# stdstu12/YUME

Hardware: AMD Instinct MI355X
Metric: denoise-steps/sec (Yume-5B 720P, 33-frame latent) (higher is better)
Workload: dtype bf16; 1 GPU; Yume-5B-720P random-init, 33-frame 704x1280 clip (latent 48x13x44x80, FramePack lfz=8, L=9460), ODE Euler steps of a 50-step shift-7 schedule, no CFG, one chain per GPU; num_layers=30, parallelism=dp1 (independent chains, replicated weights)

## Files before the change

### include/yume_hip.h

```cpp
#ifndef YUME_HIP_H
#define YUME_HIP_H

#include <stdint.h>

#ifdef __cplusplus
extern "C" {
#endif

#define YUME_OK 0
#define YUME_EINVAL (-1)
#define YUME_ELAUNCH (-2)
#define YUME_EUNSUP (-3)

const char* yume_last_error(void);
#define YUME_ABI_VERSION 9
int yume_abi_version(void);
const char* yume_target_arch(void);

int64_t yume_counter_workspace_bytes(void);
int yume_counter_workspace_init(void* ptr, int64_t bytes, void* stream);

int yume_calibrate_mfma(int64_t iters, int64_t workgroups, void* ticks, void* sink, void* stream);

int yume_adaln_modulate(const float* x, int64_t ldx, int64_t T, int64_t C, float eps,
// ... 13 lines not shown
};
int yume_gemm_bf16(const void* A, int64_t lda, const void* W, int64_t ldw, const float* bias,
                   int64_t M, int64_t N, int64_t K, int epi,
                   void* out, int64_t ldo,
                   const float* gate, int64_t gate_stride, const int32_t* row_idx,
                   void* outT, int64_t ldt, int64_t n_split,
                   int variant, void* stream);

int64_t yume_gemm_workspace_bytes(void);
int yume_gemm_bf16_ws(const void* A, int64_t lda, const void* W, int64_t ldw, const float* bias,
                      int64_t M, int64_t N, int64_t K, int epi,
                      void* out, int64_t ldo,
                      const float* gate, int64_t gate_stride, const int32_t* row_idx,
                      void* outT, int64_t ldt, int64_t n_split,
                      int variant, void* workspace, int64_t workspace_bytes, void* stream);

int yume_quant_rows_e4m3(const void* x, int64_t ldx, int64_t R, int64_t K, void* q, int64_t ldq, float* scale, void* stream);
int yume_gemm_f8(const void* Aq, int64_t lda, const float* sa, const void* Wq, int64_t ldw, const float* sw,
                 const float* bias, int64_t M, int64_t N, int64_t K, int epi, void* out, int64_t ldo,
                 const float* gate, int64_t gate_stride, const int32_t* row_idx, void* stream);
int yume_gemm_f8_splitt(const void* Aq, int64_t lda, const float* sa, const void* Wq, int64_t ldw, const float* sw,
                        const float* bias, int64_t M, int64_t N, int64_t K,
                        void* out, int64_t ldo, void* outT, int64_t ldt, int64_t n_split, void* stream);

int yume_adaln_modulate_e4m3(const float* x, int64_t ldx, int64_t T, int64_t C, float eps, const float* mul,
                             const float* add, int64_t tab_stride, const int32_t* row_idx, int add_one,
                             void* q, int64_t ldq, float* scale, void* stream);
int yume_gemm_f8_mxout(const void* Aq, int64_t lda, const float* sa, const void* Wq, int64_t ldw, const float* sw,
                       const float* bias, int64_t M, int64_t N, int64_t K, int epi, void* out, int64_t ldo,
                       void* eo, int64_t ldeo, void* stream);
int yume_gemm_f8_mx(const void* Aq, int64_t lda, const void* ea, int64_t ldea, const void* Wq, int64_t ldw, const float* sw,
                    const float* bias, int64_t M, int64_t N, int64_t K, int epi, void* out, int64_t ldo,
                    const float* gate, int64_t gate_stride, const int32_t* row_idx, void* stream);

int yume_rmsnorm_rope(void* buf, int64_t ld, int64_t T, int64_t C, int nparts,
                      const float* w, float eps, const float* rope, int64_t D, void* stream);
int yume_rmsnorm_rows_periodic(void* buf, int64_t ld, int64_t T, int64_t C, const float* w, int64_t wperiod, float eps,
                               void* stream);

#define YUME_ATTN_Q_PRESCALED 0x100
#define YUME_ATTN_KV_PADDED 0x200
int yume_attn_fwd(const void* Q, int64_t ldq, const void* K, int64_t ldk, const void* Vt, int64_t ldvt,
                  void* O, int64_t ldo, int64_t Lq, int64_t Lk, int64_t H, float scale,
                  int accumulate, int variant, void* stream);
int64_t yume_attn_workspace_bytes(int64_t Lq, int64_t Lk, int64_t H);
int yume_attn_fwd_ws(const void* Q, int64_t ldq, const void* K, int64_t ldk, const void* Vt, int64_t ldvt,
                     void* O, int64_t ldo, int64_t Lq, int64_t Lk, int64_t H, float scale,
                     int accumulate, int variant, void* workspace, int64_t workspace_bytes, void* stream);
int yume_attn_fwd_kw(const void* Q, int64_t ldq, const void* K, int64_t ldk, const void* Vt, int64_t ldvt,
                     void* O, int64_t ldo, int64_t Lq, int64_t Lk, int64_t H, float scale,
                     int accumulate, int variant, void* workspace, int64_t workspace_bytes, float last_key_weight, void* stream);
int yume_attn_fwd_seg(const void* Q, int64_t ldq, const void* const* K, int64_t ldk, const void* const* Vt, int64_t ldvt,
                      void* O, int64_t ldo, int64_t nseg, int64_t Lq_seg, int64_t seg_pitch, const int64_t* Lk, int64_t H,
                      float scale, int accumulate, int variant, const float* last_key_weight, void* stream);
int64_t yume_attn_batch_workspace_bytes(int64_t nseg, int64_t Lq_seg, int64_t Lk_seg, int64_t H);
int yume_attn_fwd_batch(const void* Q, int64_t ldq, const void* K, int64_t ldk, const void* Vt, int64_t ldvt,
                        void* O, int64_t ldo, int64_t nseg, int64_t Lq_seg, int64_t q_pitch,
                        int64_t Lk_seg, int64_t k_pitch, int64_t H, float scale, int accumulate, int variant,
                        void* workspace, int64_t workspace_bytes, void* stream);

int yume_linear_smallm_f32(const float* in, int64_t R, int64_t K, const void* W, int w_bf16,
                           const float* bias, int64_t N, int in_act, int out_act,
                           const float* add_table, float* out, void* stream);

int yume_sinusoidal_embed(const double* t, const int32_t* t_index, int64_t R, int64_t dim,
                          float* out, void* stream);
// ... 59 lines not shown
```

### yume_amd/_lib.py

```python
import ctypes
import os
from ctypes import c_void_p, c_int, c_int64, c_float, c_char_p

_HERE = os.path.dirname(os.path.abspath(__file__))
LIB_PATH = os.environ.get("YUME_HIP_LIB") or os.path.join(_HERE, "lib", "libyume_hip.so")

_P, _I, _L, _F = c_void_p, c_int, c_int64, c_float

SIGNATURES = {
    "yume_last_error": [],
    "yume_abi_version": [],
    "yume_target_arch": [],
    "yume_counter_workspace_bytes": [],
    "yume_counter_workspace_init": [_P, _L, _P],
    "yume_calibrate_mfma": [_L, _L, _P, _P, _P],
    "yume_adaln_modulate": [_P, _L, _L, _L, _F, _P, _P, _L, _P, _I, _P, _L, _I, _P],
    "yume_adaln_modulate_e4m3": [_P, _L, _L, _L, _F, _P, _P, _L, _P, _I, _P, _L, _P, _P],
    "yume_gemm_bf16": [_P, _L, _P, _L, _P, _L, _L, _L, _I, _P, _L, _P, _L, _P, _P, _L, _L, _I, _P],
    "yume_gemm_workspace_bytes": [],
    "yume_gemm_bf16_ws": [_P, _L, _P, _L, _P, _L, _L, _L, _I, _P, _L, _P, _L, _P, _P, _L, _L, _I, _P, _L, _P],
    "yume_quant_rows_e4m3": [_P, _L, _L, _L, _P, _L, _P, _P],
    "yume_gemm_f8": [_P, _L, _P, _P, _L, _P, _P, _L, _L, _L, _I, _P, _L, _P, _L, _P, _P],
    "yume_gemm_f8_splitt": [_P, _L, _P, _P, _L, _P, _P, _L, _L, _L, _P, _L, _P, _L, _L, _P],
    "yume_gemm_f8_mxout": [_P, _L, _P, _P, _L, _P, _P, _L, _L, _L, _I, _P, _L, _P, _L, _P],
    "yume_gemm_f8_mx": [_P, _L, _P, _L, _P, _L, _P, _P, _L, _L, _L, _I, _P, _L, _P, _L, _P, _P],
    "yume_rmsnorm_f32": [_P, _L, _L, _L, _F, _P, _P, _L, _P],
    "yume_gemm_bf16_batched": [_P, _L, _L, _P, _L, _L, _L, _L, _L, _I, _P, _L, _L, _L, _I, _P],
    "yume_gemm_splitk_workspace_bytes": [_L, _L, _I],
    "yume_gemm_bf16_splitk": [_P, _L, _P, _L, _P, _L, _L, _L, _I, _P, _L, _I, _P, _P],
    "yume_softmax_bias_rows": [_P, _L, _L, _L, _L, _P, _L, _P, _L, _L, _P],
    "yume_rmsnorm_rows_periodic": [_P, _L, _L, _L, _P, _L, _F, _P],
    "yume_rmsnorm_rope": [_P, _L, _L, _L, _I, _P, _F, _P, _L, _P],
    "yume_attn_fwd": [_P, _L, _P, _L, _P, _L, _P, _L, _L, _L, _L, _F, _I, _I, _P],
    "yume_attn_workspace_bytes": [_L, _L, _L],
    "yume_attn_fwd_ws": [_P, _L, _P, _L, _P, _L, _P, _L, _L, _L, _L, _F, _I, _I, _P, _L, _P],
    "yume_attn_fwd_kw": [_P, _L, _P, _L, _P, _L, _P, _L, _L, _L, _L, _F, _I, _I, _P, _L, _F, _P],
    "yume_attn_fwd_seg": [_P, _L, _P, _L, _P, _L, _P, _L, _L, _L, _L, _P, _L, _F, _I, _I, _P, _P],
    "yume_attn_batch_workspace_bytes": [_L, _L, _L, _L],
    "yume_attn_fwd_batch": [_P, _L, _P, _L, _P, _L, _P, _L, _L, _L, _L, _L, _L, _L, _F, _I, _I, _P, _L, _P],
    "yume_linear_smallm_f32": [_P, _L, _L, _P, _I, _P, _L, _I, _I, _P, _P, _P],
    "yume_sinusoidal_embed": [_P, _P, _L, _L, _P, _P],
    "yume_modulation_table": [_P, _P, _L, _L, _L, _P, _P],
    "yume_patch_gather": [_P, _I, _L, _L, _L, _L, _L, _L, _L, _L, _P, _L, _P],
    "yume_unpatchify": [_P, _L, _L, _L, _L, _L, _L, _L, _P, _P],
    "yume_cast_bf16": [_P, _L, _L, _L, _L, _P, _L, _P],
    "yume_transpose_bf16": [_P, _I, _L, _L, _L, _P, _L, _P],
    "yume_conv3d_cl": [_P, _P, _L, _L, _L, _L, _L, _P, _L, _P, _L, _I, _I, _I, _I, _I, _I, _I, _I, _I, _I, _L, _L, _L, _I, _P, _L,
                       _P, _L, _P, _P],
    "yume_vae_rmsnorm_silu": [_P, _L, _L, _L, _P, _P, _I, _P, _L, _P],
    "yume_vae_dupup_add": [_P, _L, _L, _L, _L, _L, _P, _L, _L, _L, _I, _I, _I, _P],
    "yume_vae_avgdown_add": [_P, _L, _L, _L, _L, _L, _P, _L, _L, _I, _I, _P],
    "yume_softmax_rows": [_P, _L, _L, _L, _F, _P, _L, _P],
    "yume_vae_pack_input": [_P, _I, _L, _L, _L, _L, _I, _P, _P, _P, _L, _P],
    "yume_frames_u8": [_P, _L, _L, _L, _L, _P, _P],
    "yume_frames_u8_trunc": [_P, _L, _L, _L, _L, _P, _P],
    "yume_vae_unpack_output": [_P, _L, _L, _L, _L, _L, _I, _P, _P, _F, _F, _P, _P],
}
_RES = {"yume_last_error": c_char_p, "yume_target_arch": c_char_p, "yume_gemm_splitk_workspace_bytes": c_int64, "yume_attn_workspace_bytes": c_int64,
# ... 35 lines not shown
```

### yume_amd/csrc/gemm_f8.hip

```cpp
#include "gemm_f8.hpp"

using namespace gemm_core;

namespace {
bool f8_log() {
    static const bool on = [] { const char* v = getenv("YUME_GEMM_LOG"); return v && atoi(v) != 0; }();
    return on;
}
}

extern "C" int yume_gemm_f8(const void* Aq, int64_t lda, const float* sa, const void* Wq, int64_t ldw, const float* sw, const float* bias,
                            int64_t M, int64_t N, int64_t K, int epi, void* out, int64_t ldo, const float* gate, int64_t gate_stride,
                            const int32_t* row_idx, void* stream) {
    if (epi != YUME_EPI_BF16 && epi != YUME_EPI_BF16_GELU && epi != YUME_EPI_F32 && epi != YUME_EPI_RESID) {
        yume_set_error("gemm_f8: epilogue %d is not implemented (BF16, GELU, F32, RESID are)", epi);
        return YUME_EUNSUP;
    }
    YUME_REQUIRE(Aq && Wq && sa && sw && out, "gemm_f8: NULL pointer");
    YUME_REQUIRE(M > 0 && N > 0 && K > 0, "gemm_f8: empty problem M=%lld N=%lld K=%lld", (long long)M, (long long)N, (long long)K);
    YUME_REQUIRE(M < (1ll << 31) && N < (1ll << 31) && K < (1ll << 31), "gemm_f8: dimension too large");
    YUME_REQUIRE((K % gemm_f8::F8_BK) == 0, "gemm_f8: K=%lld must be a multiple of %d", (long long)K, gemm_f8::F8_BK);
    YUME_REQUIRE((N % 4) == 0, "gemm_f8: N=%lld must be a multiple of 4", (long long)N);
    YUME_REQUIRE((lda % 16) == 0 && (ldw % 16) == 0 && lda >= K && ldw >= K, "gemm_f8: lda/ldw must be multiples of 16 (16-byte rows) and >= K");
    YUME_REQUIRE((ldo % 4) == 0 && ldo >= N, "gemm_f8: ldo must be a multiple of 4 and >= N");
    YUME_REQUIRE(((uintptr_t)Aq % 16) == 0 && ((uintptr_t)Wq % 16) == 0 && ((uintptr_t)out % 16) == 0 && ((uintptr_t)sw % 16) == 0 &&
                 ((uintptr_t)sa % 4) == 0 && (bias == nullptr || ((uintptr_t)bias % 16) == 0),
                 "gemm_f8: Aq, Wq, out, sw and bias must be 16-byte aligned");
    if (epi == YUME_EPI_RESID)
        YUME_REQUIRE(gate == nullptr || ((gate_stride % 4) == 0 && ((uintptr_t)gate % 16) == 0), "gemm_f8: gate must be 16-byte aligned, gate_stride a multiple of 4");
    Problem p = {};
    p.M = (int)M; p.N = (int)N; p.K = (int)K;
    gemm_f8::F8Args f = {};
    f.A = (const unsigned char*)Aq; f.lda = lda; f.sa = sa;
    f.W = (const unsigned char*)Wq; f.ldw = ldw; f.sw = sw;
    Epilogue e = {};
    e.bias = bias;
    e.out = out; e.ldo = ldo;
    e.gate = gate; e.gate_stride = gate_stride; e.row_idx = row_idx;
    if (f8_log())
        fprintf(stderr, "[gemm_f8] f8 M=%lld N=%lld K=%lld epi=%d lda=%lld ldw=%lld ldo=%lld\n", (long long)M, (long long)N, (long long)K, epi,
                (long long)lda, (long long)ldw, (long long)ldo);
    return gemm_f8::launch_f8(epi, p, f, e, (hipStream_t)stream);
}

extern "C" int yume_gemm_f8_splitt(const void* Aq, int64_t lda, const float* sa, const void* Wq, int64_t ldw, const float* sw, const float* bias,
                                   int64_t M, int64_t N, int64_t K, void* out, int64_t ldo, void* outT, int64_t ldt, int64_t n_split,
                                   void* stream) {
    YUME_REQUIRE(Aq && Wq && sa && sw, "gemm_f8_splitt: NULL pointer");
    YUME_REQUIRE(M > 0 && N > 0 && K > 0, "gemm_f8_splitt: empty problem M=%lld N=%lld K=%lld", (long long)M, (long long)N, (long long)K);
    YUME_REQUIRE(M < (1ll << 31) && N < (1ll << 31) && K < (1ll << 31), "gemm_f8_splitt: dimension too large");
    YUME_REQUIRE((K % gemm_f8::F8_BK) == 0, "gemm_f8_splitt: K=%lld must be a multiple of %d", (long long)K, gemm_f8::F8_BK);
    YUME_REQUIRE((N % 4) == 0, "gemm_f8_splitt: N=%lld must be a multiple of 4", (long long)N);
    YUME_REQUIRE((lda % 16) == 0 && (ldw % 16) == 0 && lda >= K && ldw >= K, "gemm_f8_splitt: lda/ldw must be multiples of 16 (16-byte rows) and >= K");
    YUME_REQUIRE(n_split >= 0 && n_split <= N && (n_split % 256) == 0, "gemm_f8_splitt: n_split=%lld must be a multiple of 256 in [0, N=%lld]",
                 (long long)n_split, (long long)N);
    YUME_REQUIRE(n_split == 0 || out != nullptr, "gemm_f8_splitt: NULL out with n_split > 0");
    YUME_REQUIRE(n_split == 0 || ((ldo % 4) == 0 && ldo >= n_split), "gemm_f8_splitt: ldo=%lld must be a multiple of 4 and >= n_split", (long long)ldo);
    YUME_REQUIRE(n_split == N || outT != nullptr, "gemm_f8_splitt: NULL outT with n_split < N");
    YUME_REQUIRE(n_split == N || ((ldt % 8) == 0 && ldt >= M), "gemm_f8_splitt: ldt=%lld must be a multiple of 8 and >= M", (long long)ldt);
    YUME_REQUIRE(((uintptr_t)Aq % 16) == 0 && ((uintptr_t)Wq % 16) == 0 && ((uintptr_t)out % 16) == 0 && ((uintptr_t)outT % 16) == 0 &&
                 ((uintptr_t)sw % 16) == 0 && ((uintptr_t)sa % 4) == 0 && (bias == nullptr || ((uintptr_t)bias % 16) == 0),
                 "gemm_f8_splitt: Aq, Wq, out, outT, sw and bias must be 16-byte aligned");
    Problem p = {};
    p.M = (int)M; p.N = (int)N; p.K = (int)K;
    gemm_f8::F8Args f = {};
    f.A = (const unsigned char*)Aq; f.lda = lda; f.sa = sa;
    f.W = (const unsigned char*)Wq; f.ldw = ldw; f.sw = sw;
    Epilogue e = {};
    e.bias = bias;
    e.out = out; e.ldo = ldo;
    e.outT = (unsigned short*)outT; e.ldt = ldt; e.n_split = (int)n_split;
    if (f8_log())
        fprintf(stderr, "[gemm_f8] f8 M=%lld N=%lld K=%lld epi=%d lda=%lld ldw=%lld ldo=%lld ldt=%lld n_split=%lld\n", (long long)M, (long long)N,
                (long long)K, (int)YUME_EPI_BF16_SPLITT, (long long)lda, (long long)ldw, (long long)ldo, (long long)ldt, (long long)n_split);
    return gemm_f8::launch_f8(YUME_EPI_BF16_SPLITT, p, f, e, (hipStream_t)stream);
}

extern "C" int yume_gemm_f8_mxout(const void* Aq, int64_t lda, const float* sa, const void* Wq, int64_t ldw, const float* sw, const float* bias,
                                  int64_t M, int64_t N, int64_t K, int epi, void* out, int64_t ldo, void* eo, int64_t ldeo, void* stream) {
    if (epi != YUME_EPI_MX_GELU) {
        yume_set_error("gemm_f8_mxout: epilogue %d is not implemented (MX_GELU is)", epi);
        return YUME_EUNSUP;
    }
    YUME_REQUIRE(Aq && Wq && sa && sw && out && eo, "gemm_f8_mxout: NULL pointer");
    YUME_REQUIRE(M > 0 && N > 0 && K > 0, "gemm_f8_mxout: empty problem M=%lld N=%lld K=%lld", (long long)M, (long long)N, (long long)K);
    YUME_REQUIRE(M < (1ll << 31) && N < (1ll << 31) && K < (1ll << 31), "gemm_f8_mxout: dimension too large");
    YUME_REQUIRE((K % gemm_f8::F8_BK) == 0, "gemm_f8_mxout: K=%lld must be a multiple of %d", (long long)K, gemm_f8::F8_BK);
    YUME_REQUIRE((N % 32) == 0, "gemm_f8_mxout: N=%lld must be a multiple of 32 (one scale byte per 32 columns)", (long long)N);
    YUME_REQUIRE((lda % 16) == 0 && (ldw % 16) == 0 && lda >= K && ldw >= K, "gemm_f8_mxout: lda/ldw must be multiples of 16 (16-byte rows) and >= K");
    YUME_REQUIRE((ldo % 4) == 0 && ldo >= N, "gemm_f8_mxout: ldo must be a multiple of 4 and >= N");
    YUME_REQUIRE(ldeo >= N / 32, "gemm_f8_mxout: ldeo=%lld must be >= N / 32", (long long)ldeo);
    YUME_REQUIRE(((uintptr_t)Aq % 16) == 0 && ((uintptr_t)Wq % 16) == 0 && ((uintptr_t)out % 16) == 0 && ((uintptr_t)sw % 16) == 0 &&
                 ((uintptr_t)sa % 4) == 0 && (bias == nullptr || ((uintptr_t)bias % 16) == 0),
                 "gemm_f8_mxout: Aq, Wq, out, sw and bias must be 16-byte aligned");
    Problem p = {};
    p.M = (int)M; p.N = (int)N; p.K = (int)K;
    gemm_f8::F8Args f = {};
    f.A = (const unsigned char*)Aq; f.lda = lda; f.sa = sa;
    f.W = (const unsigned char*)Wq; f.ldw = ldw; f.sw = sw;
    f.eo = (unsigned char*)eo; f.ldeo = ldeo;
    Epilogue e = {};
    e.bias = bias;
    e.out = out; e.ldo = ldo;
    if (f8_log())
        fprintf(stderr, "[gemm_f8] f8 M=%lld N=%lld K=%lld epi=%d lda=%lld ldw=%lld ldo=%lld ldeo=%lld\n", (long long)M, (long long)N, (long long)K, epi,
                (long long)lda, (long long)ldw, (long long)ldo, (long long)ldeo);
    return gemm_f8::launch_f8(epi, p, f, e, (hipStream_t)stream);
}

extern "C" int yume_gemm_f8_mx(const void* Aq, int64_t lda, const void* ea, int64_t ldea, const void* Wq, int64_t ldw, const float* sw,
                               const float* bias, int64_t M, int64_t N, int64_t K, int epi, void* out, int64_t ldo, const float* gate,
                               int64_t gate_stride, const int32_t* row_idx, void* stream) {
    if (epi != YUME_EPI_F32 && epi != YUME_EPI_RESID) {
        yume_set_error("gemm_f8_mx: epilogue %d is not implemented (F32, RESID are)", epi);
        return YUME_EUNSUP;
    }
    YUME_REQUIRE(Aq && Wq && ea && sw && out, "gemm_f8_mx: NULL pointer");
    YUME_REQUIRE(M > 0 && N > 0 && K > 0, "gemm_f8_mx: empty problem M=%lld N=%lld K=%lld", (long long)M, (long long)N, (long long)K);
    YUME_REQUIRE(M < (1ll << 31) && N < (1ll << 31) && K < (1ll << 31), "gemm_f8_mx: dimension too large");
    YUME_REQUIRE((K % gemm_f8::F8_BK) == 0, "gemm_f8_mx: K=%lld must be a multiple of %d", (long long)K, gemm_f8::F8_BK);
    YUME_REQUIRE((N % 4) == 0, "gemm_f8_mx: N=%lld must be a multiple of 4", (long long)N);
    YUME_REQUIRE((lda % 16) == 0 && (ldw % 16) == 0 && lda >= K && ldw >= K, "gemm_f8_mx: lda/ldw must be multiples of 16 (16-byte rows) and >= K");
    YUME_REQUIRE((ldea % 16) == 0 && ldea >= K / 32, "gemm_f8_mx: ldea=%lld must be a multiple of 16 and >= K / 32", (long long)ldea);
    YUME_REQUIRE((ldo % 4) == 0 && ldo >= N, "gemm_f8_mx: ldo must be a multiple of 4 and >= N");
    YUME_REQUIRE(((uintptr_t)Aq % 16) == 0 && ((uintptr_t)Wq % 16) == 0 && ((uintptr_t)out % 16) == 0 && ((uintptr_t)sw % 16) == 0 &&
                 ((uintptr_t)ea % 16) == 0 && (bias == nullptr || ((uintptr_t)bias % 16) == 0),
                 "gemm_f8_mx: Aq, ea, Wq, out, sw and bias must be 16-byte aligned");
    if (epi == YUME_EPI_RESID)
        YUME_REQUIRE(gate == nullptr || ((gate_stride % 4) == 0 && ((uintptr_t)gate % 16) == 0), "gemm_f8_mx: gate must be 16-byte aligned, gate_stride a multiple of 4");
    Problem p = {};
    p.M = (int)M; p.N = (int)N; p.K = (int)K;
    gemm_f8::F8Args f = {};
    f.A = (const unsigned char*)Aq; f.lda = lda;
    f.W = (const unsigned char*)Wq; f.ldw = ldw; f.sw = sw;
    f.ea = (const unsigned char*)ea; f.ldea = ldea;
    Epilogue e = {};
    e.bias = bias;
    e.out = out; e.ldo = ldo;
    e.gate = gate; e.gate_stride = gate_stride; e.row_idx = row_idx;
    if (f8_log())
        fprintf(stderr, "[gemm_f8] mx M=%lld N=%lld K=%lld epi=%d lda=%lld ldea=%lld ldw=%lld ldo=%lld\n", (long long)M, (long long)N, (long long)K, epi,
                (long long)lda, (long long)ldea, (long long)ldw, (long long)ldo);
    return gemm_f8::launch_f8_mx(epi, p, f, e, (hipStream_t)stream);
}
```

### yume_amd/csrc/gemm_f8.hpp

```cpp
#pragma once
#include "gemm_w4.hpp"

namespace gemm_f8 {
using namespace gemm_core;

typedef __attribute__((ext_vector_type(8))) int i32x8;

constexpr int F8_BK = 128;
constexpr int F8_NTHR = 256;
constexpr int F8_OPER = 256 * F8_BK;
constexpr int F8_BUF = 2 * F8_OPER;
constexpr int F8_LDS = 2 * F8_BUF;

struct F8Args {
    const unsigned char* A; int64_t lda; const float* sa;
    const unsigned char* W; int64_t ldw; const float* sw;
    const unsigned char* ea; int64_t ldea;
    unsigned char* eo; int64_t ldeo;
};

constexpr int EPI_MX_GELU = YUME_EPI_MX_GELU;

__device__ __forceinline__ void f8_stage(const unsigned char* const (&ga)[8], const unsigned char* const (&gw)[8], int koff, char* buf, int wave) {
#pragma unroll
// ... 143 lines not shown
                for (int h = 0; h < 2; ++h) {
                    float t[4];
#pragma unroll
                    for (int c = 0; c < 4; ++c) t[c] = fminf(fmaxf(v[h][c] * mult, -448.0f), 448.0f);
                    int w = __builtin_amdgcn_cvt_pk_fp8_f32(t[0], t[1], 0, false);
                    w = __builtin_amdgcn_cvt_pk_fp8_f32(t[2], t[3], w, true);
                    *reinterpret_cast<int*>(qo + (int64_t)m * e.ldo + nb + 16 * h + 4 * l4) = w;
                }
                if (l4 == 0) f.eo[(int64_t)m * f.ldeo + (nb >> 5)] = (unsigned char)byte;
            }
        }
    }
}

__device__ __forceinline__ i32x8 f8_frag_mx(const char* oper, int row, int lane) {
    const int q = lane >> 4;
    const char* rp = oper + row * F8_BK;
    const u32x4 lo = *reinterpret_cast<const u32x4*>(rp + (((q ^ row) & 7) << 4));
    const u32x4 hi = *reinterpret_cast<const u32x4*>(rp + ((((4 + q) ^ row) & 7) << 4));
    return i32x8{(int)lo[0], (int)lo[1], (int)lo[2], (int)lo[3], (int)hi[0], (int)hi[1], (int)hi[2], (int)hi[3]};
}

__device__ __forceinline__ void f8_mx_scales_load(const unsigned char* const (&ge)[8], int g, u32x4 (&raw)[8]) {
#pragma unroll
    for (int i = 0; i < 8; ++i) raw[i] = *reinterpret_cast<const u32x4*>(ge[i] + 16 * g);
}
__device__ __forceinline__ void f8_mx_scales_pack(const u32x4 (&raw)[8], int lane, unsigned (&pk)[8]) {
    const int sh = 8 * (lane >> 4);
#pragma unroll
    for (int i = 0; i < 8; ++i)
        pk[i] = ((raw[i][0] >> sh) & 0xffu) | (((raw[i][1] >> sh) & 0xffu) << 8) | (((raw[i][2] >> sh) & 0xffu) << 16) | ((raw[i][3] >> sh) << 24 & 0xff000000u);
}

template <int EPI>
__global__ __launch_bounds__(F8_NTHR, 1) void gemm_f8_mx_kernel(Problem p, F8Args f, Epilogue e) {
    __shared__ __attribute__((aligned(16))) char smem[F8_LDS];
    const int tid = threadIdx.x;
    const int lane = tid & 63;
    const int wave = __builtin_amdgcn_readfirstlane(tid >> 6);
    const int wr = wave >> 1, wc = wave & 1;
    int start, count, m0, n0;
    xcd_chunk(p.tiles_m * p.tiles_n, blockIdx.x & 7, start, count);
    tile_origin(p, start + (blockIdx.x >> 3), m0, n0);

    const unsigned char* ga[8];
    const unsigned char* gw[8];
    const unsigned char* ge[8];
    {
        const int rl = 8 * wave + (lane >> 3);
#pragma unroll
        for (int j = 0; j < 8; ++j) {
            const int r = 32 * j + rl;
            const int ch = ((lane & 7) ^ (r & 7)) << 4;
            ga[j] = f.A + (int64_t)min(m0 + r, p.M - 1) * f.lda + ch;
            gw[j] = f.W + (int64_t)min(n0 + r, p.N - 1) * f.ldw + ch;
        }
#pragma unroll
        for (int i = 0; i < 8; ++i) ge[i] = f.ea + (int64_t)min(m0 + wr * 128 + 16 * i + (lane & 15), p.M - 1) * f.ldea;
    }
    f32x4 acc[8][8];
#pragma unroll
    for (int i = 0; i < 8; ++i)
#pragma unroll
        for (int j = 0; j < 8; ++j) acc[i][j] = f32x4{0.f, 0.f, 0.f, 0.f};

    const int nk = p.K / F8_BK;
    u32x4 raw[8];
    unsigned pk[8], pkn[8];
    f8_mx_scales_load(ge, 0, raw);
    f8_stage(ga, gw, 0, smem, wave);
    f8_mx_scales_pack(raw, lane, pk);
#pragma unroll
    for (int i = 0; i < 8; ++i) pkn[i] = pk[i];
    int cur = 0;
    for (int kt = 0; kt < nk; ++kt) {
        asm volatile("s_waitcnt vmcnt(0)" ::: "memory");
        __syncthreads();
        const int t = kt & 3;
        if (t == 3) f8_mx_scales_pack(raw, lane, pkn);
        if (t == 2 && kt + 2 < nk) f8_mx_scales_load(ge, (kt >> 2) + 1, raw);
        if (kt + 1 < nk) f8_stage(ga, gw, (kt + 1) * F8_BK, smem + (cur ^ 1) * F8_BUF, wave);
        const char* At = smem + cur * F8_BUF;
        const char* Wt = At + F8_OPER;
        i32x8 a[8];
        int sc[8];
#pragma unroll
        for (int i = 0; i < 8; ++i) {
            a[i] = f8_frag_mx(At, wr * 128 + 16 * i + (lane & 15), lane);
            sc[i] = (int)(pk[i] >> (8 * t));
        }
#pragma unroll
        for (int j = 0; j < 8; ++j) {
            const i32x8 w = f8_frag_mx(Wt, wc * 128 + 16 * j + (lane & 15), lane);
#pragma unroll
            for (int i = 0; i < 8; ++i)
                acc[i][j] = __builtin_amdgcn_mfma_scale_f32_16x16x128_f8f6f4(w, a[i], acc[i][j], 0, 0, 0, 0x7f7f7f7f, 0, sc[i]);
        }
        if (t == 3) {
#pragma unroll
            for (int i = 0; i < 8; ++i) pk[i] = pkn[i];
        }
        cur ^= 1;
    }
    f8_epilogue<EPI, true>(acc, p, f, e, m0, n0, smem);
}

template <int EPI>
__global__ __launch_bounds__(F8_NTHR, 1) void gemm_f8_kernel(Problem p, F8Args f, Epilogue e) {
    __shared__ __attribute__((aligned(16))) char smem[F8_LDS];
    const int tid = threadIdx.x;
    const int lane = tid & 63;
    const int wave = __builtin_amdgcn_readfirstlane(tid >> 6);
    const int wr = wave >> 1, wc = wave & 1;
    int start, count, m0, n0;
    xcd_chunk(p.tiles_m * p.tiles_n, blockIdx.x & 7, start, count);
    tile_origin(p, start + (blockIdx.x >> 3), m0, n0);

    const unsigned char* ga[8];
    const unsigned char* gw[8];
    {
        const int rl = 8 * wave + (lane >> 3);
#pragma unroll
        for (int j = 0; j < 8; ++j) {
            const int r = 32 * j + rl;
            const int ch = ((lane & 7) ^ (r & 7)) << 4;
            ga[j] = f.A + (int64_t)min(m0 + r, p.M - 1) * f.lda + ch;
            gw[j] = f.W + (int64_t)min(n0 + r, p.N - 1) * f.ldw + ch;
        }
    }
    f32x4 acc[8][8];
#pragma unroll
    for (int i = 0; i < 8; ++i)
#pragma unroll
        for (int j = 0; j < 8; ++j) acc[i][j] = f32x4{0.f, 0.f, 0.f, 0.f};

    const int nk = p.K / F8_BK;
    f8_stage(ga, gw, 0, smem, wave);
    int cur = 0;
    for (int kt = 0; kt < nk; ++kt) {
        asm volatile("s_waitcnt vmcnt(0)" ::: "memory");
        __syncthreads();
        if (kt + 1 < nk) f8_stage(ga, gw, (kt + 1) * F8_BK, smem + (cur ^ 1) * F8_BUF, wave);
        const char* At = smem + cur * F8_BUF;
        const char* Wt = At + F8_OPER;
        i32x8 a[8];
#pragma unroll
        for (int i = 0; i < 8; ++i) a[i] = f8_frag(At, wr * 128 + 16 * i + (lane & 15), lane);
#pragma unroll
        for (int j = 0; j < 8; ++j) {
            const i32x8 w = f8_frag(Wt, wc * 128 + 16 * j + (lane & 15), lane);
#pragma unroll
            for (int i = 0; i < 8; ++i)
                acc[i][j] = __builtin_amdgcn_mfma_scale_f32_16x16x128_f8f6f4(w, a[i], acc[i][j], 0, 0, 0, 0x7f7f7f7f, 0, 0x7f7f7f7f);
        }
        cur ^= 1;
    }
    if constexpr (EPI == EPI_MX_GELU) f8_epilogue_mx_gelu(acc, p, f, e, m0, n0);
    else f8_epilogue<EPI>(acc, p, f, e, m0, n0, smem);
}

inline int launch_f8(int epi, Problem p, const F8Args& f, const Epilogue& e, hipStream_t st) {
    p.tiles_m = (p.M + 255) / 256;
    p.tiles_n = (p.N + 255) / 256;
    p.group_m = g_group_m;
    const dim3 grid((unsigned)(p.tiles_m * p.tiles_n)), block(F8_NTHR);
    switch (epi) {
        case YUME_EPI_BF16_GELU: hipLaunchKernelGGL(gemm_f8_kernel<YUME_EPI_BF16_GELU>, grid, block, 0, st, p, f, e); break;
        case YUME_EPI_F32: hipLaunchKernelGGL(gemm_f8_kernel<YUME_EPI_F32>, grid, block, 0, st, p, f, e); break;
        case YUME_EPI_RESID: hipLaunchKernelGGL(gemm_f8_kernel<YUME_EPI_RESID>, grid, block, 0, st, p, f, e); break;
        case EPI_MX_GELU: hipLaunchKernelGGL(gemm_f8_kernel<EPI_MX_GELU>, grid, block, 0, st, p, f, e); break;
        case YUME_EPI_BF16_SPLITT: hipLaunchKernelGGL(gemm_f8_kernel<YUME_EPI_BF16_SPLITT>, grid, block, 0, st, p, f, e); break;
        default: hipLaunchKernelGGL(gemm_f8_kernel<YUME_EPI_BF16>, grid, block, 0, st, p, f, e); break;
    }
    YUME_CHECK_LAUNCH("gemm_f8");
    return YUME_OK;
}

inline int launch_f8_mx(int epi, Problem p, const F8Args& f, const Epilogue& e, hipStream_t st) {
    p.tiles_m = (p.M + 255) / 256;
    p.tiles_n = (p.N + 255) / 256;
    p.group_m = g_group_m;
    const dim3 grid((unsigned)(p.tiles_m * p.tiles_n)), block(F8_NTHR);
    if (epi == YUME_EPI_RESID) hipLaunchKernelGGL(gemm_f8_mx_kernel<YUME_EPI_RESID>, grid, block, 0, st, p, f, e);
    else hipLaunchKernelGGL(gemm_f8_mx_kernel<YUME_EPI_F32>, grid, block, 0, st, p, f, e);
    YUME_CHECK_LAUNCH("gemm_f8_mx");
    return YUME_OK;
}

}
```

### yume_amd/ops.py

```python
import math
import os

import torch

from . import _lib

EPI_BF16, EPI_BF16_GELU, EPI_F32, EPI_RESID, EPI_BF16_SPLITT, EPI_BF16_GELU_ERF, EPI_BF16_GEGLU = 0, 1, 2, 3, 4, 5, 6


def _stream():
    return torch.cuda.current_stream().cuda_stream


def _dev(t, name, dtype=None):
    if not isinstance(t, torch.Tensor) or t.device.type != "cuda":
        raise RuntimeError(f"yume_amd: {name} must be a device ('cuda') tensor — this path has no CPU fallback")
    if dtype is not None and t.dtype != dtype:
        raise RuntimeError(f"yume_amd: {name} must be {dtype}, got {t.dtype}")
    return t


def _rows(t, name):
    if t.dim() != 2 or t.stride(1) != 1:
        raise RuntimeError(f"yume_amd: {name} must be 2-D with a contiguous last dim, got shape {tuple(t.shape)} stride {t.stride()}")
# ... 168 lines not shown


def gemm_f8_splitt(aq, sa, wq, sw, bias, out, out_t, n_split):
    lib = _lib.load()
    _dev(aq, "aq", torch.uint8)
    _dev(wq, "wq", torch.uint8)
    _dev(sa, "sa", torch.float32)
    _dev(sw, "sw", torch.float32)
    ap, lda = _rows(aq, "aq")
    wp, ldw = _rows(wq, "wq")
    M, K = aq.shape
    N, K2 = wq.shape
    if K != K2:
        raise RuntimeError(f"yume_amd.gemm_f8_splitt: K mismatch {K} vs {K2}")
    if sa.dim() != 1 or sa.numel() != M or not sa.is_contiguous() or sw.dim() != 1 or sw.numel() != N or not sw.is_contiguous():
        raise RuntimeError(f"yume_amd.gemm_f8_splitt: scales sa {tuple(sa.shape)}, sw {tuple(sw.shape)} do not fit M={M}, N={N}")
    op, ldo, tp, ldt = None, 0, None, 0
    if out is not None:
        _dev(out, "out", torch.bfloat16)
        op, ldo = _rows(out, "out")
        if out.shape[0] < M or out.shape[1] < n_split:
            raise RuntimeError(f"yume_amd.gemm_f8_splitt: out {tuple(out.shape)} does not hold [{M}, {n_split}]")
    if out_t is not None:
        _dev(out_t, "out_t", torch.bfloat16)
        tp, ldt = _rows(out_t, "out_t")
        if out_t.shape[0] < N - n_split:
            raise RuntimeError(f"yume_amd.gemm_f8_splitt: out_t {tuple(out_t.shape)} does not hold {N - n_split} rows")
    rc = lib.yume_gemm_f8_splitt(ap, lda, sa.data_ptr(), wp, ldw, sw.data_ptr(), _ptr(bias), M, N, K, op, ldo, tp, ldt, n_split, _stream())
    _lib.check(rc, "yume_gemm_f8_splitt")
    return out, out_t


EPI_MX_GELU = 7


def gemm_f8_mxout(aq, sa, wq, sw, bias, out, eo, epi=EPI_MX_GELU):
    lib = _lib.load()
    _dev(aq, "aq", torch.uint8)
    _dev(wq, "wq", torch.uint8)
    _dev(sa, "sa", torch.float32)
    _dev(sw, "sw", torch.float32)
    _dev(out, "out", torch.uint8)
    _dev(eo, "eo", torch.uint8)
    ap, lda = _rows(aq, "aq")
    wp, ldw = _rows(wq, "wq")
    M, K = aq.shape
    N, K2 = wq.shape
    if K != K2:
        raise RuntimeError(f"yume_amd.gemm_f8_mxout: K mismatch {K} vs {K2}")
    if sa.dim() != 1 or sa.numel() != M or not sa.is_contiguous() or sw.dim() != 1 or sw.numel() != N or not sw.is_contiguous():
        raise RuntimeError(f"yume_amd.gemm_f8_mxout: scales sa {tuple(sa.shape)}, sw {tuple(sw.shape)} do not fit M={M}, N={N}")
    op, ldo = _rows(out, "out")
    ep, ldeo = _rows(eo, "eo")
    if tuple(out.shape) != (M, N) or tuple(eo.shape) != (M, N // 32):
        raise RuntimeError(f"yume_amd.gemm_f8_mxout: out {tuple(out.shape)}, eo {tuple(eo.shape)} do not fit M={M}, N={N}")
    rc = lib.yume_gemm_f8_mxout(ap, lda, sa.data_ptr(), wp, ldw, sw.data_ptr(), _ptr(bias), M, N, K, epi, op, ldo, ep, ldeo, _stream())
    _lib.check(rc, "yume_gemm_f8_mxout")
    return out, eo


def gemm_f8_mx(aq, ea, wq, sw, bias, out, epi=EPI_F32, gate=None, gate_stride=0, row_idx=None):
    lib = _lib.load()
    _dev(aq, "aq", torch.uint8)
    _dev(wq, "wq", torch.uint8)
    _dev(ea, "ea", torch.uint8)
    _dev(sw, "sw", torch.float32)
# ... 291 lines not shown
```

Measured before the change: 10.27 denoise-steps/sec.

## Add hand-scheduled FP8 GEMM main loop interleaving MFMA with LDS DMA

Adds an alternative main loop for the FP8 and MX GEMM kernels that statically schedules 32 MFMA slots per K-step. Global-to-LDS DMA loads, barriers, scale loads and LDS operand reads are placed between the MFMAs using inline assembly. It is on by default, can be turned off with the YUME_GEMM_F8_LOOP environment variable or a new API call, and falls back to the old loop when offsets would overflow 32 bits. The goal is to hide memory and LDS latency behind matrix math better than the compiler-scheduled loop does. The cost is fragile hand-written assembly with manual waitcnt and barrier placement, which risks hazards or correctness bugs.

```diff
diff --git a/include/yume_hip.h b/include/yume_hip.h
--- a/include/yume_hip.h
+++ b/include/yume_hip.h
@@ -69,6 +69,7 @@
 int yume_gemm_f8_mx(const void* Aq, int64_t lda, const void* ea, int64_t ldea, const void* Wq, int64_t ldw, const float* sw,
                     const float* bias, int64_t M, int64_t N, int64_t K, int epi, void* out, int64_t ldo,
                     const float* gate, int64_t gate_stride, const int32_t* row_idx, void* stream);
+int yume_gemm_f8_loop(int mode);
 
 int yume_rmsnorm_rope(void* buf, int64_t ld, int64_t T, int64_t C, int nparts,
                       const float* w, float eps, const float* rope, int64_t D, void* stream);
diff --git a/yume_amd/_lib.py b/yume_amd/_lib.py
--- a/yume_amd/_lib.py
+++ b/yume_amd/_lib.py
@@ -24,6 +24,7 @@
     "yume_gemm_f8_splitt": [_P, _L, _P, _P, _L, _P, _P, _L, _L, _L, _P, _L, _P, _L, _L, _P],
     "yume_gemm_f8_mxout": [_P, _L, _P, _P, _L, _P, _P, _L, _L, _L, _I, _P, _L, _P, _L, _P],
     "yume_gemm_f8_mx": [_P, _L, _P, _L, _P, _L, _P, _P, _L, _L, _L, _I, _P, _L, _P, _L, _P, _P],
+    "yume_gemm_f8_loop": [_I],
     "yume_rmsnorm_f32": [_P, _L, _L, _L, _F, _P, _P, _L, _P],
     "yume_gemm_bf16_batched": [_P, _L, _L, _P, _L, _L, _L, _L, _L, _I, _P, _L, _L, _L, _I, _P],
     "yume_gemm_splitk_workspace_bytes": [_L, _L, _I],
diff --git a/yume_amd/csrc/gemm_f8.hip b/yume_amd/csrc/gemm_f8.hip
--- a/yume_amd/csrc/gemm_f8.hip
+++ b/yume_amd/csrc/gemm_f8.hip
@@ -7,6 +7,30 @@
     static const bool on = [] { const char* v = getenv("YUME_GEMM_LOG"); return v && atoi(v) != 0; }();
     return on;
 }
+
+int g_f8_loop = -1;
+int f8_loop_mode() {
+    if (g_f8_loop < 0) {
+        const char* v = getenv("YUME_GEMM_F8_LOOP");
+        g_f8_loop = (v && atoi(v) == 0) ? 0 : 1;
+    }
+    return g_f8_loop;
+}
+bool f8_hand() {
+    const bool hand = f8_loop_mode() == 1;
+    static bool said = false;
+    if (!said && f8_log()) {
+        said = true;
+        fprintf(stderr, "[f8_loop] %s\n", hand ? "hand" : "reference");
+    }
+    return hand;
+}
+}
+
+extern "C" int yume_gemm_f8_loop(int mode) {
+    const int prev = f8_loop_mode();
+    if (mode == 0 || mode == 1) g_f8_loop = mode;
+    return prev;
 }
 
 extern "C" int yume_gemm_f8(const void* Aq, int64_t lda, const float* sa, const void* Wq, int64_t ldw, const float* sw, const float* bias,
@@ -40,7 +64,7 @@
     if (f8_log())
         fprintf(stderr, "[gemm_f8] f8 M=%lld N=%lld K=%lld epi=%d lda=%lld ldw=%lld ldo=%lld\n", (long long)M, (long long)N, (long long)K, epi,
                 (long long)lda, (long long)ldw, (long long)ldo);
-    return gemm_f8::launch_f8(epi, p, f, e, (hipStream_t)stream);
+    return gemm_f8::launch_f8(epi, p, f, e, (hipStream_t)stream, f8_hand());
 }
 
 extern "C" int yume_gemm_f8_splitt(const void* Aq, int64_t lda, const float* sa, const void* Wq, int64_t ldw, const float* sw, const float* bias,
@@ -73,7 +97,7 @@
     if (f8_log())
         fprintf(stderr, "[gemm_f8] f8 M=%lld N=%lld K=%lld epi=%d lda=%lld ldw=%lld ldo=%lld ldt=%lld n_split=%lld\n", (long long)M, (long long)N,
                 (long long)K, (int)YUME_EPI_BF16_SPLITT, (long long)lda, (long long)ldw, (long long)ldo, (long long)ldt, (long long)n_split);
-    return gemm_f8::launch_f8(YUME_EPI_BF16_SPLITT, p, f, e, (hipStream_t)stream);
+    return gemm_f8::launch_f8(YUME_EPI_BF16_SPLITT, p, f, e, (hipStream_t)stream, f8_hand());
 }
 
 extern "C" int yume_gemm_f8_mxout(const void* Aq, int64_t lda, const float* sa, const void* Wq, int64_t ldw, const float* sw, const float* bias,
@@ -105,7 +129,7 @@
     if (f8_log())
         fprintf(stderr, "[gemm_f8] f8 M=%lld N=%lld K=%lld epi=%d lda=%lld ldw=%lld ldo=%lld ldeo=%lld\n", (long long)M, (long long)N, (long long)K, epi,
                 (long long)lda, (long long)ldw, (long long)ldo, (long long)ldeo);
-    return gemm_f8::launch_f8(epi, p, f, e, (hipStream_t)stream);
+    return gemm_f8::launch_f8(epi, p, f, e, (hipStream_t)stream, f8_hand());
 }
 
 extern "C" int yume_gemm_f8_mx(const void* Aq, int64_t lda, const void* ea, int64_t ldea, const void* Wq, int64_t ldw, const float* sw,
@@ -141,5 +165,5 @@
     if (f8_log())
         fprintf(stderr, "[gemm_f8] mx M=%lld N=%lld K=%lld epi=%d lda=%lld ldea=%lld ldw=%lld ldo=%lld\n", (long long)M, (long long)N, (long long)K, epi,
                 (long long)lda, (long long)ldea, (long long)ldw, (long long)ldo);
-    return gemm_f8::launch_f8_mx(epi, p, f, e, (hipStream_t)stream);
+    return gemm_f8::launch_f8_mx(epi, p, f, e, (hipStream_t)stream, f8_hand());
 }
diff --git a/yume_amd/csrc/gemm_f8.hpp b/yume_amd/csrc/gemm_f8.hpp
--- a/yume_amd/csrc/gemm_f8.hpp
+++ b/yume_amd/csrc/gemm_f8.hpp
@@ -199,7 +199,196 @@
         pk[i] = ((raw[i][0] >> sh) & 0xffu) | (((raw[i][1] >> sh) & 0xffu) << 8) | (((raw[i][2] >> sh) & 0xffu) << 16) | ((raw[i][3] >> sh) << 24 & 0xff000000u);
 }
 
-template <int EPI>
+struct HCtx {
+    char* smem;
+    i32x8 a[8], w[8];
+    unsigned cw_lo, cw_hi, na_lo, na_hi, nw_lo, nw_hi;
+    unsigned va[8], vb[8];
+    const char* pa;
+    const char* pb;
+    unsigned lcur;
+    unsigned one;
+    unsigned ve[8], raw[8], sc[8], sh;
+    const char* pe;
+};
+
+#define F8H_MFMA "v_mfma_scale_f32_16x16x128_f8f6f4 "
+#define F8H_MFMA2(C0, C1, W0, W1, A, SW, SA)                                                                                            \
+    asm volatile(F8H_MFMA "%0, %2, %4, %0, %5, %6 op_sel_hi:[0,0,0]\n\t" F8H_MFMA "%1, %3, %4, %1, %5, %6 op_sel_hi:[0,0,0]"                 \
+                 : "+a"(C0), "+a"(C1) : "v"(W0), "v"(W1), "v"(A), "v"(SW), "v"(SA) : "memory")
+#define F8H_MFMA2_DMA(C0, C1, W0, W1, A, SW, SA, voff, sbase, lbase, loff)                                                               \
+    asm volatile("s_add_u32 m0, %9, %10\n\t" F8H_MFMA "%0, %2, %4, %0, %5, %6 op_sel_hi:[0,0,0]\n\tglobal_load_lds_dwordx4 %7, %8\n\t"     \
+                 F8H_MFMA "%1, %3, %4, %1, %5, %6 op_sel_hi:[0,0,0]"                                                                   \
+                 : "+a"(C0), "+a"(C1) : "v"(W0), "v"(W1), "v"(A), "v"(SW), "v"(SA), "v"(voff), "s"(sbase), "s"(lbase), "n"(loff) : "memory", "scc")
+#define F8H_LOFF(q) (((q) >> 3) * F8_OPER + ((q) & 7) * 4096)
+
+constexpr int FH_BAR_A = 5;
+constexpr int FH_SCALES = 6;
+constexpr int FH_DMA0 = 7;
+constexpr int FH_BAR_B = 17;
+constexpr int fh_dma_pos(int q) { return FH_DMA0 + (q * (31 - FH_DMA0)) / 15; }
+constexpr int fh_piece_at(int s) {
+    for (int q = 0; q < 16; ++q)
+        if (fh_dma_pos(q) == s) return q;
+    return -1;
+}
+constexpr int fh_pieces_before_bar_b() {
+    int k = 0;
+    for (int q = 0; q < 16; ++q) k += fh_dma_pos(q) <= FH_BAR_B ? 1 : 0;
+    return k;
+}
+constexpr int fh_next_read(int s) {
+    switch (s) {
+        case 18: return 0;  case 19: return 8;  case 20: return 1;  case 21: return 9;  case 22: return 2;  case 23: return 10;
+        case 24: return 3;  case 25: return 11; case 26: return 12; case 28: return 13; case 30: return 14; case 31: return 15;
+        default: return -1;
+    }
+}
+static_assert(fh_dma_pos(0) > FH_BAR_A && fh_dma_pos(0) > FH_SCALES && fh_dma_pos(15) == 31, "the plan must fit the 32 slots");
+
+__device__ __forceinline__ i32x8 f8h_read(const HCtx& c, unsigned lo_off, unsigned hi_off, int idx) {
+    const u32x4 lo = *reinterpret_cast<const u32x4*>(c.smem + lo_off + idx * 2048);
+    const u32x4 hi = *reinterpret_cast<const u32x4*>(c.smem + hi_off + idx * 2048);
+    return i32x8{(int)lo[0], (int)lo[1], (int)lo[2], (int)lo[3], (int)hi[0], (int)hi[1], (int)hi[2], (int)hi[3]};
+}
+
+__device__ __forceinline__ void f8h_scale_loads(HCtx& c) {
+    asm volatile("global_load_dword %0, %8, %16\n\tglobal_load_dword %1, %9, %16\n\tglobal_load_dword %2, %10, %16\n\tglobal_load_dword %3, %11, %16\n\t"
+                 "global_load_dword %4, %12, %16\n\tglobal_load_dword %5, %13, %16\n\tglobal_load_dword %6, %14, %16\n\tglobal_load_dword %7, %15, %16"
+                 : "=&v"(c.raw[0]), "=&v"(c.raw[1]), "=&v"(c.raw[2]), "=&v"(c.raw[3]), "=&v"(c.raw[4]), "=&v"(c.raw[5]), "=&v"(c.raw[6]), "=&v"(c.raw[7])
+                 : "v"(c.ve[0]), "v"(c.ve[1]), "v"(c.ve[2]), "v"(c.ve[3]), "v"(c.ve[4]), "v"(c.ve[5]), "v"(c.ve[6]), "v"(c.ve[7]), "s"(c.pe) : "memory");
+}
+template <int KEEP, bool MX>
+__device__ __forceinline__ void f8h_wait(HCtx& c) {
+    if constexpr (MX)
+        asm volatile("s_waitcnt vmcnt(%c8)\n\ts_barrier" : "+v"(c.raw[0]), "+v"(c.raw[1]), "+v"(c.raw[2]), "+v"(c.raw[3]), "+v"(c.raw[4]), "+v"(c.raw[5]),
+                     "+v"(c.raw[6]), "+v"(c.raw[7]) : "n"(KEEP) : "memory");
+    else asm volatile("s_waitcnt vmcnt(%c0)\n\ts_barrier" ::"n"(KEEP) : "memory");
+}
+
+template <int s, bool DMA, bool MX>
+__device__ __forceinline__ void f8h_slots(HCtx& c, f32x4 (&acc)[8][8]) {
+    if constexpr (s < 32) {
+        constexpr int i = (s & 15) >> 1, j = 4 * (s >> 4) + 2 * (s & 1);
+        constexpr int q = DMA ? fh_piece_at(s) : -1;
+        const unsigned sa = MX ? c.sc[i] : c.one;
+        if constexpr (q >= 0 && q < 8) F8H_MFMA2_DMA(acc[i][j], acc[i][j + 1], c.w[j], c.w[j + 1], c.a[i], c.one, sa, c.va[q & 7], c.pa, c.lcur, F8H_LOFF(q & 15));
+        else if constexpr (q >= 8) F8H_MFMA2_DMA(acc[i][j], acc[i][j + 1], c.w[j], c.w[j + 1], c.a[i], c.one, sa, c.vb[q & 7], c.pb, c.lcur, F8H_LOFF(q & 15));
+        else F8H_MFMA2(acc[i][j], acc[i][j + 1], c.w[j], c.w[j + 1], c.a[i], c.one, sa);
+        if constexpr (s < 4) c.w[4 + s] = f8h_read(c, c.cw_lo, c.cw_hi, 4 + s);
+        if constexpr (s == FH_BAR_A) asm volatile("s_waitcnt lgkmcnt(0)\n\ts_barrier" ::: "memory");
+        if constexpr (MX && s == FH_SCALES) f8h_scale_loads(c);
+        if constexpr (s == FH_BAR_B) f8h_wait<DMA ? fh_pieces_before_bar_b() : 0, MX>(c);
+        constexpr int r = fh_next_read(s);
+        if constexpr (r >= 8) c.a[r & 7] = f8h_read(c, c.na_lo, c.na_hi, r & 7);
+        else if constexpr (r >= 0) c.w[r & 7] = f8h_read(c, c.nw_lo, c.nw_hi, r & 7);
+        f8h_slots<s + 1, DMA, MX>(c, acc);
+    }
+}
+
+template <int q>
+__device__ __forceinline__ void f8h_stage_all(HCtx& c) {
+    if constexpr (q < 16) {
+        if constexpr (q < 8) W4_DMA(c.va[q & 7], c.pa, c.lcur, F8H_LOFF(q));
+        else W4_DMA(c.vb[q & 7], c.pb, c.lcur, F8H_LOFF(q));
+        f8h_stage_all<q + 1>(c);
+    }
+}
+
+template <bool DMA, bool MX>
+__device__ __forceinline__ void f8h_loop(HCtx& c, f32x4 (&acc)[8][8], int t0, int t1, int nk, unsigned lbase) {
+    for (int t = t0; t < t1; ++t) {
+        f8h_slots<0, DMA, MX>(c, acc);
+        if constexpr (DMA) {
+            c.pa += F8_BK;
+            c.pb += F8_BK;
+        }
+        c.lcur = lbase + (((t + 1) & 1) ? F8_BUF : 0);
+        c.cw_lo ^= F8_BUF; c.cw_hi ^= F8_BUF;
+        c.na_lo ^= F8_BUF; c.na_hi ^= F8_BUF;
+        c.nw_lo ^= F8_BUF; c.nw_hi ^= F8_BUF;
+        if constexpr (MX) {
+#pragma unroll
+            for (int i = 0; i < 8; ++i) c.sc[i] = c.raw[i] >> c.sh;
+            if (t + 2 < nk) c.pe += 4;
+        }
+    }
+}
+
+template <bool MX>
+__device__ __forceinline__ void f8h_mainloop(const Problem& p, const F8Args& f, char* smem, int m0, int n0, f32x4 (&acc)[8][8]) {
+    const int tid = threadIdx.x;
+    const int lane = tid & 63;
+    const int wave = __builtin_amdgcn_readfirstlane(tid >> 6);
+    const int wr = wave >> 1, wc = wave & 1;
+    const int l15 = lane & 15, q = lane >> 4;
+    const int nk = p.K / F8_BK;
+    HCtx c;
+    c.smem = smem;
+    c.one = 0x7f7f7f7fu;
+    asm volatile("" : "+v"(c.one));
+    const unsigned lbase = (unsigned)(uintptr_t)(__attribute__((address_space(3))) char*)smem + wave * 1024;
+    c.lcur = lbase;
+    c.pa = reinterpret_cast<const char*>(f.A) + (int64_t)m0 * f.lda;
+    c.pb = reinterpret_cast<const char*>(f.W) + (int64_t)n0 * f.ldw;
+    {
+        const int rl = 8 * wave + (lane >> 3);
+        const unsigned ch = (unsigned)(((lane & 7) ^ (rl & 7)) << 4);
+        const int mleft = p.M - 1 - m0, nleft = p.N - 1 - n0;
+#pragma unroll
+        for (int j = 0; j < 8; ++j) {
+            const int r = 32 * j + rl;
+            c.va[j] = (unsigned)min(r, mleft) * (unsigned)f.lda + ch;
+            c.vb[j] = (unsigned)min(r, nleft) * (unsigned)f.ldw + ch;
+        }
+    }
+    const unsigned plo = (unsigned)((((MX ? q : 2 * q) ^ l15) & 7) << 4), phi = plo ^ (MX ? 64u : 16u);
+    const unsigned rowa = (unsigned)((wr * 128 + l15) * F8_BK), roww = (unsigned)(F8_OPER + (wc * 128 + l15) * F8_BK);
+    if constexpr (MX) {
+        c.sh = 8u * (unsigned)q;
+        c.pe = reinterpret_cast<const char*>(f.ea);
+#pragma unroll
+        for (int i = 0; i < 8; ++i) c.ve[i] = (unsigned)min(m0 + wr * 128 + 16 * i + l15, p.M - 1) * (unsigned)f.ldea;
+        f8h_scale_loads(c);
+        if (nk > 1) c.pe += 4;
+    }
+    f8h_stage_all<0>(c);
+    if (nk > 1) { c.pa += F8_BK; c.pb += F8_BK; }
+    c.lcur = lbase + F8_BUF;
+    f8h_stage_all<0>(c);
+    c.pa += F8_BK;
+    c.pb += F8_BK;
+    c.lcur = lbase;
+#pragma unroll
+    for (int i = 0; i < 8; ++i)
+#pragma unroll
+        for (int j = 0; j < 8; ++j) acc[i][j] = f32x4{0.f, 0.f, 0.f, 0.f};
+    f8h_wait<16, MX>(c);
+    if constexpr (MX) {
+#pragma unroll
+        for (int i = 0; i < 8; ++i) c.sc[i] = c.raw[i] >> c.sh;
+    }
+#pragma unroll
+    for (int r = 0; r < 8; ++r) {
+        if (r < 4) c.w[r] = f8h_read(c, roww + plo, roww + phi, r);
+        c.a[r] = f8h_read(c, rowa + plo, rowa + phi, r);
+    }
+    c.cw_lo = roww + plo; c.cw_hi = roww + phi;
+    c.na_lo = F8_BUF + rowa + plo; c.na_hi = F8_BUF + rowa + phi;
+    c.nw_lo = F8_BUF + roww + plo; c.nw_hi = F8_BUF + roww + phi;
+    f8h_loop<true, MX>(c, acc, 0, nk - 2, nk, lbase);
+    f8h_loop<false, MX>(c, acc, max(nk - 2, 0), nk, nk, lbase);
+    asm volatile("s_nop 15\n\ts_nop 15" : "+a"(acc[6][4]), "+a"(acc[6][5]), "+a"(acc[6][6]), "+a"(acc[6][7]), "+a"(acc[7][4]), "+a"(acc[7][5]),
+                 "+a"(acc[7][6]), "+a"(acc[7][7]));
+}
+
+inline bool f8h_applies(const Problem& p, const F8Args& f) {
+    if (255ll * f.lda + 128 >= (1ll << 32) || 255ll * f.ldw + 128 >= (1ll << 32)) return false;
+    if (f.ea && (int64_t)(p.M - 1) * f.ldea + 4 >= (1ll << 32)) return false;
+    return true;
+}
+
+template <int EPI, bool HAND = false>
 __global__ __launch_bounds__(F8_NTHR, 1) void gemm_f8_mx_kernel(Problem p, F8Args f, Epilogue e) {
     __shared__ __attribute__((aligned(16))) char smem[F8_LDS];
     const int tid = threadIdx.x;
@@ -209,6 +398,12 @@
     int start, count, m0, n0;
     xcd_chunk(p.tiles_m * p.tiles_n, blockIdx.x & 7, start, count);
     tile_origin(p, start + (blockIdx.x >> 3), m0, n0);
+    if constexpr (HAND) {
+        f32x4 acc[8][8];
+        f8h_mainloop<true>(p, f, smem, m0, n0, acc);
+        f8_epilogue<EPI, true>(acc, p, f, e, m0, n0, smem);
+        return;
+    }
 
     const unsigned char* ga[8];
     const unsigned char* gw[8];
@@ -272,7 +467,7 @@
     f8_epilogue<EPI, true>(acc, p, f, e, m0, n0, smem);
 }
 
-template <int EPI>
+template <int EPI, bool HAND = false>
 __global__ __launch_bounds__(F8_NTHR, 1) void gemm_f8_kernel(Problem p, F8Args f, Epilogue e) {
     __shared__ __attribute__((aligned(16))) char smem[F8_LDS];
     const int tid = threadIdx.x;
@@ -282,6 +477,13 @@
     int start, count, m0, n0;
     xcd_chunk(p.tiles_m * p.tiles_n, blockIdx.x & 7, start, count);
     tile_origin(p, start + (blockIdx.x >> 3), m0, n0);
+    if constexpr (HAND) {
+        f32x4 acc[8][8];
+        f8h_mainloop<false>(p, f, smem, m0, n0, acc);
+        if constexpr (EPI == EPI_MX_GELU) f8_epilogue_mx_gelu(acc, p, f, e, m0, n0);
+        else f8_epilogue<EPI>(acc, p, f, e, m0, n0, smem);
+        return;
+    }
 
     const unsigned char* ga[8];
     const unsigned char* gw[8];
@@ -326,30 +528,41 @@
     else f8_epilogue<EPI>(acc, p, f, e, m0, n0, smem);
 }
 
-inline int launch_f8(int epi, Problem p, const F8Args& f, const Epilogue& e, hipStream_t st) {
+template <bool HAND>
+inline void launch_f8_as(int epi, const dim3& grid, const dim3& block, const Problem& p, const F8Args& f, const Epilogue& e, hipStream_t st) {
+    switch (epi) {
+        case YUME_EPI_BF16_GELU: hipLaunchKernelGGL((gemm_f8_kernel<YUME_EPI_BF16_GELU, HAND>), grid, block, 0, st, p, f, e); break;
+        case YUME_EPI_F32: hipLaunchKernelGGL((gemm_f8_kernel<YUME_EPI_F32, HAND>), grid, block, 0, st, p, f, e); break;
+        case YUME_EPI_RESID: hipLaunchKernelGGL((gemm_f8_kernel<YUME_EPI_RESID, HAND>), grid, block, 0, st, p, f, e); break;
+        case EPI_MX_GELU: hipLaunchKernelGGL((gemm_f8_kernel<EPI_MX_GELU, HAND>), grid, block, 0, st, p, f, e); break;
+        case YUME_EPI_BF16_SPLITT: hipLaunchKernelGGL((gemm_f8_kernel<YUME_EPI_BF16_SPLITT, HAND>), grid, block, 0, st, p, f, e); break;
+        default: hipLaunchKernelGGL((gemm_f8_kernel<YUME_EPI_BF16, HAND>), grid, block, 0, st, p, f, e); break;
+    }
+}
+
+inline int launch_f8(int epi, Problem p, const F8Args& f, const Epilogue& e, hipStream_t st, bool hand) {
     p.tiles_m = (p.M + 255) / 256;
     p.tiles_n = (p.N + 255) / 256;
     p.group_m = g_group_m;
     const dim3 grid((unsigned)(p.tiles_m * p.tiles_n)), block(F8_NTHR);
-    switch (epi) {
-        case YUME_EPI_BF16_GELU: hipLaunchKernelGGL(gemm_f8_kernel<YUME_EPI_BF16_GELU>, grid, block, 0, st, p, f, e); break;
-        case YUME_EPI_F32: hipLaunchKernelGGL(gemm_f8_kernel<YUME_EPI_F32>, grid, block, 0, st, p, f, e); break;
-        case YUME_EPI_RESID: hipLaunchKernelGGL(gemm_f8_kernel<YUME_EPI_RESID>, grid, block, 0, st, p, f, e); break;
-        case EPI_MX_GELU: hipLaunchKernelGGL(gemm_f8_kernel<EPI_MX_GELU>, grid, block, 0, st, p, f, e); break;
-        case YUME_EPI_BF16_SPLITT: hipLaunchKernelGGL(gemm_f8_kernel<YUME_EPI_BF16_SPLITT>, grid, block, 0, st, p, f, e); break;
-        default: hipLaunchKernelGGL(gemm_f8_kernel<YUME_EPI_BF16>, grid, block, 0, st, p, f, e); break;
-    }
+    if (hand && f8h_applies(p, f)) launch_f8_as<true>(epi, grid, block, p, f, e, st);
+    else launch_f8_as<false>(epi, grid, block, p, f, e, st);
     YUME_CHECK_LAUNCH("gemm_f8");
     return YUME_OK;
 }
 
-inline int launch_f8_mx(int epi, Problem p, const F8Args& f, const Epilogue& e, hipStream_t st) {
+inline int launch_f8_mx(int epi, Problem p, const F8Args& f, const Epilogue& e, hipStream_t st, bool hand) {
     p.tiles_m = (p.M + 255) / 256;
     p.tiles_n = (p.N + 255) / 256;
     p.group_m = g_group_m;
     const dim3 grid((unsigned)(p.tiles_m * p.tiles_n)), block(F8_NTHR);
-    if (epi == YUME_EPI_RESID) hipLaunchKernelGGL(gemm_f8_mx_kernel<YUME_EPI_RESID>, grid, block, 0, st, p, f, e);
-    else hipLaunchKernelGGL(gemm_f8_mx_kernel<YUME_EPI_F32>, grid, block, 0, st, p, f, e);
+    if (hand && f8h_applies(p, f)) {
+        if (epi == YUME_EPI_RESID) hipLaunchKernelGGL((gemm_f8_mx_kernel<YUME_EPI_RESID, true>), grid, block, 0, st, p, f, e);
+        else hipLaunchKernelGGL((gemm_f8_mx_kernel<YUME_EPI_F32, true>), grid, block, 0, st, p, f, e);
+    } else {
+        if (epi == YUME_EPI_RESID) hipLaunchKernelGGL((gemm_f8_mx_kernel<YUME_EPI_RESID, false>), grid, block, 0, st, p, f, e);
+        else hipLaunchKernelGGL((gemm_f8_mx_kernel<YUME_EPI_F32, false>), grid, block, 0, st, p, f, e);
+    }
     YUME_CHECK_LAUNCH("gemm_f8_mx");
     return YUME_OK;
 }
diff --git a/yume_amd/ops.py b/yume_amd/ops.py
--- a/yume_amd/ops.py
+++ b/yume_amd/ops.py
@@ -224,6 +224,10 @@
 
 
 EPI_MX_GELU = 7
+
+
+def gemm_f8_loop(mode=-1):
+    return int(_lib.load().yume_gemm_f8_loop(int(mode)))
 
 
 def gemm_f8_mxout(aq, sa, wq, sw, bias, out, eo, epi=EPI_MX_GELU):
```

New measurement: 10.26 denoise-steps/sec, median of 2. No clear change (-0.1%).
